# ArtyZe/yolo_quantization

Hardware: AMD Instinct MI355X
Metric: images/sec yolov3-tiny INT8 416x416 (higher is better)
Workload: dtype u8 x s8 -> int32 (f64 or exact-integer requant, bit-identical); 1 GPU; yolov3-tiny full net (cfg/yolov3-tiny_quant.cfg, leaky, per-channel quant), batch 64/GPU synthetic uint8 416x416, inputs resident in HBM (NCHW uint8); global_batch=64, parallelism=image-sharded x1, RCCL weight broadcast once, batches_in_flight=4, kernel_plan=throughput (kernels of which two workgroups share a CU)

## Files before the change

yolo_quantization_amd/csrc/conv_pool16.hip:

```cpp
#include "kargs.h"
#include <cstdlib>
#include <type_traits>

constexpr int P16_PITCH = 40;
constexpr int P16_HC = 20;
constexpr int P16_NDMA = 12;
constexpr int P16_PLANEB = P16_NDMA * 1024;

#define P16_DMA(ldsdst_u32, sbase_ptr, voff_u32)                                                                  \
    asm volatile("s_mov_b32 m0, %0\n\ts_nop 0\n\tglobal_load_lds_dwordx4 %1, %2" ::"s"(ldsdst_u32), "v"(voff_u32), \
                 "s"(sbase_ptr)                                                                                  \
                 : "memory", "m0")

template <int ACT, bool SAT>
__global__ __launch_bounds__(256, 3) void conv_pool16_kernel(const ConvArgs a)
{
    constexpr int C = 16, NM = 2, KS = 3, N = 16 * NM;
    constexpr int BUFB = P16_PLANEB;
    constexpr bool LUT = ACT == MI355_ACT_LEAKY && !SAT;
    constexpr bool INTRQ = LUT || ACT == MI355_ACT_RELU6;
    __shared__ __attribute__((aligned(16))) char img[2 * BUFB];
    __shared__ __attribute__((aligned(16))) uint8_t lut[LUT ? LUTQ_N : 16];
    __shared__ __attribute__((aligned(16))) int ldsCB[N], ldsHI[N], ldsLO[N], ldsM0[N], ldsSH[N], ldsDZ[N];
    __shared__ __attribute__((aligned(16))) double ldsMP[INTRQ ? 2 : N];

    const int tid = threadIdx.x;
    const int lane = tid & 63;
    const int wave = __builtin_amdgcn_readfirstlane(tid >> 6);
    const int pc = lane & 15, g = lane >> 4;
    const int W1 = a.W + 1;
    const int OH = a.H >> 1, OW = a.W >> 1;
    const int tiles_x = (OW + 15) >> 4, tiles_y = (OH + 7) >> 3, tpi = tiles_x * tiles_y;
    const int ntiles = a.B * tpi;
    const unsigned lds0 = (unsigned)(size_t)(__attribute__((address_space(3))) char *)img;

    int relc[3];
#pragma unroll
    for (int i = 0; i < 3; ++i) {
        const int q = 64 * (wave + 4 * i) + lane;
        const int r = min(q / P16_PITCH, 17), sl = q % P16_PITCH;
        const int half = sl >= P16_HC ? 1 : 0, ci = min(2 * (sl - P16_HC * half) + half, 33);
        relc[i] = r * W1 + ci;
    }
    const int maxcell = a.in_cells - 1;
    auto issue_tile = [&](unsigned org, int buf) {
#pragma unroll
        for (int i = 0; i < 3; ++i) {
            const int f = min(max((int)org + relc[i], 0), maxcell);
            const unsigned voff = (unsigned)f * (unsigned)C;
            const unsigned d = lds0 + (unsigned)buf * BUFB + (unsigned)(wave + 4 * i) * 1024u;
            P16_DMA(d, a.x, voff);
        }
    };

    const bool xcd_walk = (gridDim.x & 7) == 0 && !(a.debug & 2048);
    const int per_x = xcd_walk ? (ntiles + 7) >> 3 : ntiles;
    const int tstride = xcd_walk ? (int)(gridDim.x >> 3) : (int)gridDim.x;
    const int tbase_x = xcd_walk ? (int)(blockIdx.x & 7) * per_x : 0;
    const int tend = min(tbase_x + per_x, ntiles);
    const int tile0 = tbase_x + (xcd_walk ? (int)(blockIdx.x >> 3) : (int)blockIdx.x);
    unsigned T_in, T_out, T_fl;
    int nt;
    {
        const int t = tile0 + lane * tstride;
        nt = __builtin_popcountll(__builtin_amdgcn_ballot_w64(t < tend));
        const int tc = min(t, ntiles - 1);
        const int b = fd_div(tc, a.fd_hw);
        const int r = tc - b * tpi;
        const int ty = fd_div(r, a.fd_w), tx = r - ty * tiles_x;
        T_in = (unsigned)(a.in_lead + (b * (a.H + 1) + 16 * ty) * W1 + 32 * tx - 1);
        T_out = (unsigned)(a.pool_lead + (b * (OH + 1) + 8 * ty + 1) * (OW + 1) + 16 * tx) * (unsigned)a.pool_cs;
        const bool tall = 16 * tx + 16 <= OW && 8 * ty + 8 <= OH;
        T_fl = (tall ? 2u : 0u) | ((unsigned)tx << 2) | ((unsigned)ty << 12);
    }
    auto tile_word = [&](unsigned v, int k) { return (unsigned)__builtin_amdgcn_readlane((int)v, k); };

    if (nt > 0) issue_tile(tile_word(T_in, 0), 0);

    const bool ept_ok = a.ept != nullptr && a.ept->key == ept_key(ACT, a.zp_act);
    const uint32_t eflags = ept_ok ? a.ept->flags : (EPT_NEVER | EPT_NOINT);
    const bool pow2 = a.hdr->pow2 == 1;
    const bool fast = ept_ok && pow2 && !(eflags & EPT_NEVER) && (!INTRQ || !(eflags & EPT_NOINT));
    if (tid < N) {
        int cbv = a.cwb[tid], hiv = 0, lov = 0, m0v = 0, shv = 0;
        if (ept_ok) {
            const EptEntry e = reinterpret_cast<const EptEntry *>(a.ept + 1)[tid];
            cbv = e.cbl; hiv = (int)e.rg; lov = e.lb; m0v = e.m0; shv = e.sh;
        }
        ldsCB[tid] = cbv; ldsHI[tid] = hiv; ldsLO[tid] = lov; ldsM0[tid] = m0v; ldsSH[tid] = shv;
        ldsDZ[tid] = a.dzp[tid];
        if (!INTRQ) ldsMP[tid] = a.mprime[tid];
    }
    if constexpr (LUT) {
        if (ept_ok) {
            const uint32_t *src = reinterpret_cast<const uint32_t *>(reinterpret_cast<const EptEntry *>(a.ept + 1) + a.hdr->mpad);
#pragma unroll
            for (int k = 0; k < LUTQ_N / 4 / 256; ++k) reinterpret_cast<uint32_t *>(lut)[tid + 256 * k] = src[tid + 256 * k];
        }
    }
    v4i wa[NM][KS], ones[KS];
    int tapk[KS];
#pragma unroll
    for (int ks = 0; ks < KS; ++ks) {
        const int t = 4 * ks + g;
        tapk[ks] = t > 8 ? 8 : t;
        const int o = t <= 8 ? 0x01010101 : 0;
        ones[ks] = v4i{o, o, o, o};
#pragma unroll
        for (int mt = 0; mt < NM; ++mt)
            wa[mt][ks] = *reinterpret_cast<const v4i *>(a.wp + ((size_t)(mt * KS + ks) * 1024) + g * 256 + pc * 16);
    }

    unsigned baddr[KS][2];
#pragma unroll
    for (int ks = 0; ks < KS; ++ks) {
        const int dy = tapk[ks] / 3, dx = tapk[ks] - 3 * dy;
#pragma unroll
        for (int jx = 0; jx < 2; ++jx) {
            const int e = jx + dx;
            baddr[ks][jx] = (unsigned)(((4 * wave + dy) * P16_PITCH + pc + (e & 1) * P16_HC + (e >> 1)) * 16);
        }
    }

    const unsigned rowpitch = (unsigned)(OW + 1) * (unsigned)a.pool_cs;
    unsigned d_out = 0;
#ifndef MI355_NARROW_STORES
    const unsigned st_off = (unsigned)(2 * wave + (g >> 1)) * rowpitch + (unsigned)pc * (unsigned)a.pool_cs + 16u * (unsigned)(g & 1);
    uint32_t dpk[2][NM];
    v4i dq = v4i{0, 0, 0, 0};
    bool dvalid = false;
    auto transpose_dpk = [&]() {
        const auto p01 = __builtin_amdgcn_permlane16_swap(dpk[0][0], dpk[0][1], false, false);
        const auto p23 = __builtin_amdgcn_permlane16_swap(dpk[1][0], dpk[1][1], false, false);
        const auto q02 = __builtin_amdgcn_permlane32_swap(p01[0], p23[0], false, false);
        const auto q13 = __builtin_amdgcn_permlane32_swap(p01[1], p23[1], false, false);
        dq = v4i{(int)q02[0], (int)q13[0], (int)q02[1], (int)q13[1]};
    };
    auto flush_stores = [&]() {
        if (dvalid) {
            const uint64_t rp = reinterpret_cast<uint64_t>(a.ypool) + (uint64_t)d_out;
            const uint64_t rs = ((uint64_t)(uint32_t)__builtin_amdgcn_readfirstlane((int)(rp >> 32)) << 32) | (uint32_t)__builtin_amdgcn_readfirstlane((int)(uint32_t)rp);
            asm volatile("global_store_dwordx4 %0, %1, %2\n\ts_nop 1" ::"v"(st_off), "v"(dq), "s"(rs) : "memory");
        }
    };
#else
    unsigned st_off[2];
#pragma unroll
    for (int s = 0; s < 2; ++s) st_off[s] = (unsigned)(2 * wave + s) * rowpitch + (unsigned)pc * (unsigned)a.pool_cs + 4u * g;
    uint32_t dpk[2][NM];
    bool dvalid[2] = {false, false};
    auto store_patch = [&](unsigned patch_off, unsigned off, uint32_t data, auto mt_c) {
        constexpr int MT = decltype(mt_c)::value;
        const uint64_t rp = reinterpret_cast<uint64_t>(a.ypool) + (uint64_t)patch_off;
        const uint64_t rs = ((uint64_t)(uint32_t)__builtin_amdgcn_readfirstlane((int)(rp >> 32)) << 32) | (uint32_t)__builtin_amdgcn_readfirstlane((int)(uint32_t)rp);
        asm volatile("global_store_dword %0, %1, %2 offset:%3" ::"v"(off), "v"(data), "s"(rs), "n"(16 * MT) : "memory");
    };
    auto flush_stores = [&]() {
#pragma unroll
        for (int s = 0; s < 2; ++s)
            if (dvalid[s]) {
                store_patch(d_out, st_off[s], dpk[s][0], std::integral_constant<int, 0>{});
                store_patch(d_out, st_off[s], dpk[s][1], std::integral_constant<int, 1>{});
            }
    };
#endif

    unsigned fl_cur = tile_word(T_fl, 0);
    int buf = 0;
    for (int k = 0; k < nt; ++k, buf ^= 1) {
        asm volatile("s_waitcnt vmcnt(0)" ::: "memory");
        __syncthreads();
        const bool more = k + 1 < nt;
        unsigned fl_nxt = 0;
        if (more) {
            fl_nxt = tile_word(T_fl, k + 1);
            issue_tile(tile_word(T_in, k + 1), buf ^ 1);
        }
        flush_stores();
        const char *const ibp = img + (size_t)buf * BUFB;
        uint32_t margin = 0xFFFFFFFFu;
        auto load_b = [&](int s, v4i (&bf)[KS][4]) {
#pragma unroll
            for (int ks = 0; ks < KS; ++ks)
#pragma unroll
                for (int j = 0; j < 4; ++j)
                    bf[ks][j] = *reinterpret_cast<const v4i *>(ibp + baddr[ks][j & 1] + (unsigned)((2 * s + (j >> 1)) * P16_PITCH * 16));
        };
        auto chain_ones = [&](const v4i (&bf)[KS][4], v4i (&sxa)[4]) {
            __builtin_amdgcn_s_setprio(3);
#pragma unroll
            for (int j = 0; j < 4; ++j) sxa[j] = v4i{0, 0, 0, 0};
#pragma unroll
            for (int ks = 0; ks < KS; ++ks)
#pragma unroll
                for (int j = 0; j < 4; ++j) sxa[j] = __builtin_amdgcn_mfma_i32_16x16x64_i8(ones[ks], bf[ks][j], sxa[j], 0, 0, 0);
            __builtin_amdgcn_s_setprio(0);
        };
        auto chain_mt = [&](int mt, const v4i (&bf)[KS][4], const v4i &cb, v4i (&acc)[4]) {
            __builtin_amdgcn_s_setprio(3);
#pragma unroll
            for (int j = 0; j < 4; ++j) acc[j] = __builtin_amdgcn_mfma_i32_16x16x64_i8(wa[mt][0], bf[0][j], cb, 0, 0, 0);
#pragma unroll
            for (int ks = 1; ks < KS; ++ks)
#pragma unroll
                for (int j = 0; j < 4; ++j) acc[j] = __builtin_amdgcn_mfma_i32_16x16x64_i8(wa[mt][ks], bf[ks][j], acc[j], 0, 0, 0);
            __builtin_amdgcn_s_setprio(0);
        };
        auto correct = [&](v4i (&acc)[4], const v4i &dz, const v4i (&sxa)[4]) {
#pragma unroll
            for (int j = 0; j < 4; ++j)
#pragma unroll
                for (int r = 0; r < 4; ++r) acc[j][r] += __mul24(dz[r], sxa[j][0]);
        };
        if (fast) {
            v4i bf[KS][4], sxa[4];
            uint32_t bt[2][4];
            load_b(0, bf);
            v4i cb = *reinterpret_cast<const v4i *>(ldsCB + 4 * g);
#pragma unroll
            for (int q = 0; q < 4; ++q) {
                const int s = q >> 1, mt = q & 1, c0 = 16 * mt + 4 * g;
                if (mt == 0) chain_ones(bf, sxa);
                v4i acc[4];
                chain_mt(mt, bf, cb, acc);
                const v4i dz = *reinterpret_cast<const v4i *>(ldsDZ + c0);
                const v4i hi = *reinterpret_cast<const v4i *>(ldsHI + c0);
                const v4i lo = *reinterpret_cast<const v4i *>(ldsLO + c0);
                v4i m0 = v4i{0, 0, 0, 0}, sh = v4i{0, 0, 0, 0};
                if constexpr (INTRQ) {
                    m0 = *reinterpret_cast<const v4i *>(ldsM0 + c0);
                    sh = *reinterpret_cast<const v4i *>(ldsSH + c0);
                }
                if (q < 3) cb = *reinterpret_cast<const v4i *>(ldsCB + (16 * (mt ^ 1) + 4 * g));
                __builtin_amdgcn_sched_barrier(0);
                if constexpr (LUT) {
                    if (q > 0) {
                        const uint32_t pk = pack4_bytes(bt[(q - 1) & 1][0], bt[(q - 1) & 1][1], bt[(q - 1) & 1][2], bt[(q - 1) & 1][3]);
                        dpk[(q - 1) >> 1][(q - 1) & 1] = pk;
                    }
                }
                correct(acc, dz, sxa);
                uint32_t umax[4];
#pragma unroll
                for (int r = 0; r < 4; ++r) {
                    umax[r] = max(max((uint32_t)acc[0][r], (uint32_t)acc[1][r]), max((uint32_t)acc[2][r], (uint32_t)acc[3][r]));
                    margin = min(margin, __builtin_elementwise_sub_sat((uint32_t)hi[r], umax[r]));
                }
                if constexpr (INTRQ) {
                    int32_t f[4];
#pragma unroll
                    for (int r = 0; r < 4; ++r) f[r] = __mulhi((int32_t)(umax[r] + (uint32_t)lo[r]), m0[r]) >> sh[r];
                    if constexpr (LUT) {
#pragma unroll
                        for (int r = 0; r < 4; ++r) bt[q & 1][r] = lut[lutq_index(f[r])];
                    } else {
                        int32_t v[4];
#pragma unroll
                        for (int r = 0; r < 4; ++r) {
                            v[r] = a.zp_act + max(f[r], 0);
                            if (SAT) v[r] = min(v[r], 255);
                        }
                        dpk[s][mt] = pack4_biased(v[0], v[1], v[2], v[3]);
                    }
                } else {
                    int32_t amax[4][1], v1[4][1];
                    double mp4[4];
#pragma unroll
                    for (int r = 0; r < 4; ++r) {
                        amax[r][0] = (int32_t)(umax[r] + (uint32_t)lo[r]);
                        mp4[r] = ldsMP[c0 + r];
                    }
                    requant_values<ACT, SAT, 1>(amax, mp4, a.zp_act, v1);
                    dpk[s][mt] = pack4_biased(v1[0][0], v1[1][0], v1[2][0], v1[3][0]);
                }
                if (q == 1) load_b(1, bf);
                __builtin_amdgcn_sched_barrier(0);
            }
            if constexpr (LUT) dpk[1][1] = pack4_bytes(bt[1][0], bt[1][1], bt[1][2], bt[1][3]);
        }
        if (!fast || __builtin_amdgcn_ballot_w64(margin == 0u) != 0) {
#pragma unroll 1
            for (int s = 0; s < 2; ++s) {
                v4i bf[KS][4], sxa[4];
                load_b(s, bf);
                chain_ones(bf, sxa);
#pragma unroll
                for (int mt = 0; mt < NM; ++mt) {
                    const int c0 = 16 * mt + 4 * g;
                    v4i acc[4];
                    chain_mt(mt, bf, *reinterpret_cast<const v4i *>(ldsCB + c0), acc);
                    correct(acc, *reinterpret_cast<const v4i *>(ldsDZ + c0), sxa);
                    const v4i lo = *reinterpret_cast<const v4i *>(ldsLO + c0);
                    double mpr[4];
#pragma unroll
                    for (int r = 0; r < 4; ++r) mpr[r] = a.mprime[c0 + r];
                    const uint32_t packed = first_pool_exact_path<ACT, SAT>(acc, lo, mpr, a.mval + c0, a.sval + c0, a.zp_act, pow2);
                    if (s == 0) dpk[0][mt] = packed; else dpk[1][mt] = packed;
                }
            }
        }
        d_out = tile_word(T_out, k);
        {
            const int tx = (int)((fl_cur >> 2) & 1023u), ty = (int)((fl_cur >> 12) & 1023u);
            const bool all = (fl_cur & 2u) != 0;
            const bool colvalid = all || 16 * tx + pc < OW;
#ifndef MI355_NARROW_STORES
            transpose_dpk();
            dvalid = colvalid && (all || 8 * ty + 2 * wave + (g >> 1) < OH);
#else
            dvalid[0] = colvalid && (all || 8 * ty + 2 * wave < OH);
            dvalid[1] = colvalid && (all || 8 * ty + 2 * wave + 1 < OH);
#endif
        }
        fl_cur = fl_nxt;
    }
    flush_stores();
}

bool conv_pool16_eligible(int n, int c, int ksize) { return ksize == 3 && c == 16 && n == 32; }

template <int ACT>
static int p16_launch_sat(ConvArgs &a, hipStream_t st, int grid)
{
    conv_launch_note(grid, 256, 0);
    if (a.store_mode == MI355_STORE_SATURATE) hipLaunchKernelGGL((conv_pool16_kernel<ACT, true>), dim3(grid), dim3(256), 0, st, a);
    else hipLaunchKernelGGL((conv_pool16_kernel<ACT, false>), dim3(grid), dim3(256), 0, st, a);
    return hipGetLastError() == hipSuccess ? MI355_OK : MI355_EHIP;
}

int conv_pool16_launch(ConvArgs &a, hipStream_t st)
{
    const int c = a.cb * a.nchunks;
    if (!conv_pool16_eligible(a.n, c, a.ksize) || !a.ypool || a.y || a.acc_out || a.y_f32 || a.res || a.stride != 1 || !a.ept) return MI355_EINVAL;
    if ((a.H & 1) || (a.W & 1) || a.in_cs != c || a.in_lead < 1 || a.pool_w < a.n) return MI355_EINVAL;
    if ((a.pool_cs & 15) || (reinterpret_cast<uintptr_t>(a.ypool) & 15)) return MI355_EINVAL;
    if ((size_t)a.in_cells * (size_t)a.in_cs >= ((size_t)1 << 31)) return MI355_EINVAL;
    const int OH = a.H / 2, OW = a.W / 2;
    if (((long)a.pool_lead + (long)a.B * (OH + 1) * (OW + 1) + OW + 2) * a.pool_cs >= (1L << 32)) return MI355_EINVAL;
    const int tx = (OW + 15) / 16, ty = (OH + 7) / 8;
    if (tx > 1023 || ty > 1023) return MI355_EINVAL;
    const long ntiles = (long)a.B * tx * ty;
    if (ntiles >= (1L << 31)) return MI355_EINVAL;
    a.fd_w = fastdiv_make((uint32_t)tx);
    a.fd_hw = fastdiv_make((uint32_t)(tx * ty));
    a.debug = mi355_debug_flags_get();
    static const int grid_cap = getenv("MI355_P16_GRID") ? atoi(getenv("MI355_P16_GRID")) : 768;
    long g = grid_cap;
    if (ntiles < g) g = ntiles;
    const long need = (((ntiles + 7) / 8 + 63) / 64) * 8;
    if (g < need) g = need;
    if (a.act == MI355_ACT_LEAKY) return p16_launch_sat<MI355_ACT_LEAKY>(a, st, (int)g);
    if (a.act == MI355_ACT_RELU6) return p16_launch_sat<MI355_ACT_RELU6>(a, st, (int)g);
    return p16_launch_sat<MI355_ACT_LINEAR>(a, st, (int)g);
}
```

Measured before the change: 270,800 images/s.

## Compute zero-point window sums via shared box-sum MFMAs instead of per-tap ones chain

The zero-point correction needs the sum of input bytes over each 3x3 window. Previously this took a separate chain of 12 MFMAs with all-ones weights per subtile. It is now computed with 4 MFMAs over a sparse indicator matrix applied to column fragments loaded from LDS, sharing partial sums between overlapping output windows and interleaved with the mt=0 weight chain. This removes matrix-core work but adds extra LDS loads and more intricate indexing; the old path stays behind a macro.

```diff
diff --git a/yolo_quantization_amd/csrc/conv_pool16.hip b/yolo_quantization_amd/csrc/conv_pool16.hip
--- a/yolo_quantization_amd/csrc/conv_pool16.hip
+++ b/yolo_quantization_amd/csrc/conv_pool16.hip
@@ -98,14 +98,22 @@
             for (int k = 0; k < LUTQ_N / 4 / 256; ++k) reinterpret_cast<uint32_t *>(lut)[tid + 256 * k] = src[tid + 256 * k];
         }
     }
-    v4i wa[NM][KS], ones[KS];
+    v4i wa[NM][KS];
     int tapk[KS];
+#ifdef MI355_P16_ONES_CHAIN
+    v4i ones[KS];
+#else
+    const int ind = ((pc & 3) == 0 && g <= 2) || ((pc & 3) == 1 && g >= 1) ? 0x01010101 : 0;
+    const v4i boxa = v4i{ind, ind, ind, ind};
+#endif
 #pragma unroll
     for (int ks = 0; ks < KS; ++ks) {
         const int t = 4 * ks + g;
         tapk[ks] = t > 8 ? 8 : t;
+#ifdef MI355_P16_ONES_CHAIN
         const int o = t <= 8 ? 0x01010101 : 0;
         ones[ks] = v4i{o, o, o, o};
+#endif
 #pragma unroll
         for (int mt = 0; mt < NM; ++mt)
             wa[mt][ks] = *reinterpret_cast<const v4i *>(a.wp + ((size_t)(mt * KS + ks) * 1024) + g * 256 + pc * 16);
@@ -121,6 +129,10 @@
             baddr[ks][jx] = (unsigned)(((4 * wave + dy) * P16_PITCH + pc + (e & 1) * P16_HC + (e >> 1)) * 16);
         }
     }
+
+#ifndef MI355_P16_ONES_CHAIN
+    const unsigned caddr = (unsigned)(((4 * wave + ((g & 1) << 1 | g >> 1)) * P16_PITCH + pc) * 16);
+#endif
 
     const unsigned rowpitch = (unsigned)(OW + 1) * (unsigned)a.pool_cs;
     unsigned d_out = 0;
@@ -186,6 +198,7 @@
                 for (int j = 0; j < 4; ++j)
                     bf[ks][j] = *reinterpret_cast<const v4i *>(ibp + baddr[ks][j & 1] + (unsigned)((2 * s + (j >> 1)) * P16_PITCH * 16));
         };
+#ifdef MI355_P16_ONES_CHAIN
         auto chain_ones = [&](const v4i (&bf)[KS][4], v4i (&sxa)[4]) {
             __builtin_amdgcn_s_setprio(3);
 #pragma unroll
@@ -196,6 +209,29 @@
                 for (int j = 0; j < 4; ++j) sxa[j] = __builtin_amdgcn_mfma_i32_16x16x64_i8(ones[ks], bf[ks][j], sxa[j], 0, 0, 0);
             __builtin_amdgcn_s_setprio(0);
         };
+        auto sum_of = [&](const v4i (&sxa)[4], int j) { return sxa[j][0]; };
+#else
+        auto load_c = [&](int s, v4i (&cf)[4]) {
+#pragma unroll
+            for (int e = 0; e < 4; ++e)
+                cf[e] = *reinterpret_cast<const v4i *>(ibp + caddr + (unsigned)((2 * s * P16_PITCH + (e & 1) * P16_HC + (e >> 1)) * 16));
+        };
+        auto chain_mt_box = [&](const v4i (&bf)[KS][4], const v4i &cb, v4i (&acc)[4], const v4i (&cf)[4], v4i (&box)[2]) {
+            __builtin_amdgcn_s_setprio(3);
+            v4i t = __builtin_amdgcn_mfma_i32_16x16x64_i8(boxa, cf[1], v4i{0, 0, 0, 0}, 0, 0, 0);
+#pragma unroll
+            for (int j = 0; j < 4; ++j) acc[j] = __builtin_amdgcn_mfma_i32_16x16x64_i8(wa[0][0], bf[0][j], cb, 0, 0, 0);
+            t = __builtin_amdgcn_mfma_i32_16x16x64_i8(boxa, cf[2], t, 0, 0, 0);
+#pragma unroll
+            for (int j = 0; j < 4; ++j) acc[j] = __builtin_amdgcn_mfma_i32_16x16x64_i8(wa[0][1], bf[1][j], acc[j], 0, 0, 0);
+            box[0] = __builtin_amdgcn_mfma_i32_16x16x64_i8(boxa, cf[0], t, 0, 0, 0);
+            box[1] = __builtin_amdgcn_mfma_i32_16x16x64_i8(boxa, cf[3], t, 0, 0, 0);
+#pragma unroll
+            for (int j = 0; j < 4; ++j) acc[j] = __builtin_amdgcn_mfma_i32_16x16x64_i8(wa[0][2], bf[2][j], acc[j], 0, 0, 0);
+            __builtin_amdgcn_s_setprio(0);
+        };
+        auto sum_of = [&](const v4i (&box)[2], int j) { return box[j & 1][j >> 1]; };
+#endif
         auto chain_mt = [&](int mt, const v4i (&bf)[KS][4], const v4i &cb, v4i (&acc)[4]) {
             __builtin_amdgcn_s_setprio(3);
 #pragma unroll
@@ -206,23 +242,34 @@
                 for (int j = 0; j < 4; ++j) acc[j] = __builtin_amdgcn_mfma_i32_16x16x64_i8(wa[mt][ks], bf[ks][j], acc[j], 0, 0, 0);
             __builtin_amdgcn_s_setprio(0);
         };
-        auto correct = [&](v4i (&acc)[4], const v4i &dz, const v4i (&sxa)[4]) {
+        auto correct = [&](v4i (&acc)[4], const v4i &dz, const auto &sx) {
 #pragma unroll
             for (int j = 0; j < 4; ++j)
 #pragma unroll
-                for (int r = 0; r < 4; ++r) acc[j][r] += __mul24(dz[r], sxa[j][0]);
+                for (int r = 0; r < 4; ++r) acc[j][r] += __mul24(dz[r], sum_of(sx, j));
         };
         if (fast) {
-            v4i bf[KS][4], sxa[4];
+            v4i bf[KS][4];
             uint32_t bt[2][4];
             load_b(0, bf);
+#ifdef MI355_P16_ONES_CHAIN
+            v4i sx[4];
+#else
+            v4i cf[4], sx[2];
+            load_c(0, cf);
+#endif
             v4i cb = *reinterpret_cast<const v4i *>(ldsCB + 4 * g);
 #pragma unroll
             for (int q = 0; q < 4; ++q) {
                 const int s = q >> 1, mt = q & 1, c0 = 16 * mt + 4 * g;
-                if (mt == 0) chain_ones(bf, sxa);
                 v4i acc[4];
+#ifdef MI355_P16_ONES_CHAIN
+                if (mt == 0) chain_ones(bf, sx);
                 chain_mt(mt, bf, cb, acc);
+#else
+                if (mt == 0) chain_mt_box(bf, cb, acc, cf, sx);
+                else chain_mt(mt, bf, cb, acc);
+#endif
                 const v4i dz = *reinterpret_cast<const v4i *>(ldsDZ + c0);
                 const v4i hi = *reinterpret_cast<const v4i *>(ldsHI + c0);
                 const v4i lo = *reinterpret_cast<const v4i *>(ldsLO + c0);
@@ -239,7 +286,7 @@
                         dpk[(q - 1) >> 1][(q - 1) & 1] = pk;
                     }
                 }
-                correct(acc, dz, sxa);
+                correct(acc, dz, sx);
                 uint32_t umax[4];
 #pragma unroll
                 for (int r = 0; r < 4; ++r) {
@@ -273,7 +320,12 @@
                     requant_values<ACT, SAT, 1>(amax, mp4, a.zp_act, v1);
                     dpk[s][mt] = pack4_biased(v1[0][0], v1[1][0], v1[2][0], v1[3][0]);
                 }
-                if (q == 1) load_b(1, bf);
+                if (q == 1) {
+                    load_b(1, bf);
+#ifndef MI355_P16_ONES_CHAIN
+                    load_c(1, cf);
+#endif
+                }
                 __builtin_amdgcn_sched_barrier(0);
             }
             if constexpr (LUT) dpk[1][1] = pack4_bytes(bt[1][0], bt[1][1], bt[1][2], bt[1][3]);
@@ -281,15 +333,25 @@
         if (!fast || __builtin_amdgcn_ballot_w64(margin == 0u) != 0) {
 #pragma unroll 1
             for (int s = 0; s < 2; ++s) {
-                v4i bf[KS][4], sxa[4];
+                v4i bf[KS][4];
                 load_b(s, bf);
-                chain_ones(bf, sxa);
+#ifdef MI355_P16_ONES_CHAIN
+                v4i sx[4];
+                chain_ones(bf, sx);
+#else
+                v4i cf[4], sx[2];
+                load_c(s, cf);
+#endif
 #pragma unroll
                 for (int mt = 0; mt < NM; ++mt) {
                     const int c0 = 16 * mt + 4 * g;
                     v4i acc[4];
-                    chain_mt(mt, bf, *reinterpret_cast<const v4i *>(ldsCB + c0), acc);
-                    correct(acc, *reinterpret_cast<const v4i *>(ldsDZ + c0), sxa);
+#ifndef MI355_P16_ONES_CHAIN
+                    if (mt == 0) chain_mt_box(bf, *reinterpret_cast<const v4i *>(ldsCB + c0), acc, cf, sx);
+                    else
+#endif
+                        chain_mt(mt, bf, *reinterpret_cast<const v4i *>(ldsCB + c0), acc);
+                    correct(acc, *reinterpret_cast<const v4i *>(ldsDZ + c0), sx);
                     const v4i lo = *reinterpret_cast<const v4i *>(ldsLO + c0);
                     double mpr[4];
 #pragma unroll
```

New measurement: 272,200 images/s (median of 6 runs). No clear change (+0.5%).
